# CliMA/ClimateParameterizations.jl

Measured on AMD Instinct MI355X. Metric: column-timesteps/sec (fwd+adjoint), 32-level wind-mixing NDE, higher is better.
Workload: dtype f32

## Files before the change

### climateparameterizations.jl_amd/csrc/engine_regtile.hip

```cpp
#include <cstdlib>
#include "engine_regtile.h"
#include "kernel_select.h"
#include "split_bf16.h"

typedef float f32x16 __attribute__((ext_vector_type(16)));

#ifdef COLNDE_STAMPS
__device__ unsigned long long g_rt_stamps[16];
#define RT_STAMP_DECL unsigned long long rs_t0 = 0, rs_acc[8] = {0, 0, 0, 0, 0, 0, 0, 0}; const unsigned long long rs_kk = __builtin_amdgcn_s_memtime(), rs_rr = __builtin_amdgcn_s_memrealtime()
#define RT_STAMP_BEGIN() do { __builtin_amdgcn_sched_barrier(0); rs_t0 = __builtin_amdgcn_s_memtime(); __builtin_amdgcn_sched_barrier(0); } while (0)
#define RT_STAMP(i) do { __builtin_amdgcn_sched_barrier(0); unsigned long long t_ = __builtin_amdgcn_s_memtime(); rs_acc[i] += t_ - rs_t0; rs_t0 = t_; __builtin_amdgcn_sched_barrier(0); } while (0)
#define RT_STAMP_FLUSH() do { if (blockIdx.x == 0 && threadIdx.x == 0) { for (int q_ = 0; q_ < 8; q_++) g_rt_stamps[q_] = rs_acc[q_]; g_rt_stamps[8] = __builtin_amdgcn_s_memtime() - rs_kk; g_rt_stamps[9] = __builtin_amdgcn_s_memrealtime() - rs_rr; } } while (0)
#else
#define RT_STAMP_DECL
#define RT_STAMP_BEGIN()
#define RT_STAMP(i)
#define RT_STAMP_FLUSH()
#endif
typedef float f32x4v __attribute__((ext_vector_type(4)));
typedef float f32x2v __attribute__((ext_vector_type(2)));

#define RHO0(r) (((r) & 3) + 8 * ((r) >> 2))
#ifndef RT16_WAVES
#define RT16_WAVES 8
#endif
#ifndef RT_ADJ_CH
#define RT_ADJ_CH 8
#endif
#ifndef RT_ZRICH
#define RT_ZRICH 0
#endif
#ifndef RT_Z2TAPE
#define RT_Z2TAPE 0
#endif
#define RT_TAPEZ_HALF (21 * 256)
#define RT_Z2OFF ((RT_ZRICH ? 2 : 1) * RT_TAPEZ_HALF)
#define RT_TAPEZ (RT_Z2OFF + (RT_Z2TAPE ? 9 * 256 : 0))
#define RT_TAPE2 (20 * 256)

__device__ __forceinline__ f32x16 mfma32(float a, float b, f32x16 c) {
    return __builtin_amdgcn_mfma_f32_32x32x2f32(a, b, c, 0, 0, 0);
}

__device__ __forceinline__ float xchg32(float from_hi, float from_lo, int h) {
    const auto r = __builtin_amdgcn_permlane32_swap(__float_as_uint(from_hi), __float_as_uint(from_lo), false, false);
    return __uint_as_float(h ? r[0] : r[1]);
}
__device__ __forceinline__ float swap32(float x, int h) { return xchg32(x, x, h); }

__device__ __forceinline__ f32x16 shift_down(const f32x16 T, int h, float below) {
    f32x16 o;
#pragma unroll
    for (int g = 0; g < 4; g++) {
        const float recv = xchg32(g > 0 ? T[(4 * g + 15) & 15] : 0.0f, T[4 * g + 3], h);
        o[4 * g] = (h == 0 && g == 0) ? below : recv;
        o[4 * g + 1] = T[4 * g];
        o[4 * g + 2] = T[4 * g + 1];
        o[4 * g + 3] = T[4 * g + 2];
    }
    return o;
}

__device__ __forceinline__ f32x16 shift_up(const f32x16 T, int h, float above) {
    f32x16 o;
#pragma unroll
    for (int g = 0; g < 4; g++) {
        const float recv = xchg32(T[4 * g], g < 3 ? T[(4 * g + 4) & 15] : 0.0f, h);
        o[4 * g + 3] = (h == 1 && g == 3) ? above : recv;
        o[4 * g] = T[4 * g + 1];
        o[4 * g + 1] = T[4 * g + 2];
        o[4 * g + 2] = T[4 * g + 3];
    }
    return o;
}

template <int ACT>
__device__ __forceinline__ float rt_act(float z) {
    if (ACT == COLNDE_ACT_RELU) return fmaxf(z, 0.0f);
    if (ACT == COLNDE_ACT_MISH) {
        const float e = __expf(__builtin_amdgcn_fmed3f(z, -3.0e38f, 20.0f));
        const float n = e * (e + 2.0f);
        return z * fast_div(n, n + 2.0f);
    }
    if (ACT == COLNDE_ACT_SWISH) return fast_div(z, 1.0f + __expf(-z));
    if (ACT == COLNDE_ACT_TANH) { const float e = __expf(2.0f * fminf(fmaxf(z, -15.0f), 15.0f)); return 1.0f - fast_div(2.0f, 1.0f + e); }
    if (ACT == COLNDE_ACT_LEAKYRELU) return z > 0.0f ? z : 0.01f * z;
    return z;
}

template <int ACT>
__device__ __forceinline__ f32x16 act_tile(f32x16 z) {
    f32x16 o;
#pragma unroll
    for (int r = 0; r < 16; r++) o[r] = rt_act<ACT>(z[r]);
    return o;
}

struct RtBases {
    int a1[5];
    int a2;
    int a3;
};

__device__ __forceinline__ RtBases rt_bases(int lane) {
    const int i = lane & 31, h = lane >> 5;
    const int r_i = (i & 3) + 4 * (i >> 3), h_i = (i >> 2) & 1;
    RtBases b;
#pragma unroll
    for (int mt = 0; mt < 5; mt++) {
        const int G = min(mt * 16 + r_i, 74);
        const int row = (G / 25) * 50 + 2 * (G % 25) + h_i;
        b.a1[mt] = RT_W1C + row * RT_LD1 + 4 * h;
    }
    b.a2 = RT_W2C + ((r_i < 10) ? 2 * r_i + h_i : 0) * RT_LD2 + h;
    b.a3 = RT_W3C + (i - 1) * RT_LD3 + h;
    return b;
}

#define RT_SCHED_FENCE() __builtin_amdgcn_sched_barrier(0x00F)
#define RT_SCHED_HARD() __builtin_amdgcn_sched_barrier(0)

template <int N, int CH, class AF, class BF, class FF>
__device__ __forceinline__ f32x16 rt_chain_fill(const float* wl, f32x16 acc, AF aidx, BF bval, FF fill) {
    float a[2][CH];
#pragma unroll
    for (int u = 0; u < CH; u++)
        if (u < N) a[0][u] = wl[aidx(u)];
    RT_SCHED_FENCE();
#pragma unroll
    for (int c = 0; c * CH < N; c++) {
#pragma unroll
        for (int u = 0; u < CH; u++)
            if ((c + 1) * CH + u < N) a[(c + 1) & 1][u] = wl[aidx((c + 1) * CH + u)];
        fill(c);
#pragma unroll
        for (int u = 0; u < CH; u++)
            if (c * CH + u < N) acc = mfma32(a[c & 1][u], bval(c * CH + u), acc);
        RT_SCHED_FENCE();
    }
    return acc;
}

template <int N, int CH, class AF, class BF>
__device__ __forceinline__ f32x16 rt_chain(const float* wl, f32x16 acc, AF aidx, BF bval) {
    return rt_chain_fill<N, CH>(wl, acc, aidx, bval, [](int) {});
}

template <int ACT>
__device__ __forceinline__ void rt_mlp_forward(const float* wl, const RtBases& b, const f32x16 (&X)[3], int h, f32x16 (&O)[3]) {
    f32x16 A1[5];
#pragma unroll
    for (int mt = 0; mt < 5; mt++) {
        f32x16 acc;
#pragma unroll
        for (int r = 0; r < 16; r++) {
            const int G = mt * 16 + r;
            acc[r] = wl[RT_B1C + (G < 75 ? (G / 25) * 50 + 2 * (G % 25) : 150 + 2 * (G - 75)) + h];
        }
        const int base = b.a1[mt];
        A1[mt] = rt_chain_fill<48, 8>(wl, acc, [=](int s) { return base + (s >> 4) * 32 + RHO0(s & 15); },
                                      [&](int s) { return X[s >> 4][s & 15]; },
                                      [&](int c) {
                                          if (mt > 0) {
#pragma unroll
                                              for (int r = 0; r < 16; r++)
                                                  if (r / 3 == c) A1[mt > 0 ? mt - 1 : 0][r] = rt_act<ACT>(A1[mt > 0 ? mt - 1 : 0][r]);
                                          }
                                      });
    }
    f32x16 Z2[3];
#pragma unroll
    for (int n = 0; n < 3; n++) {
        f32x16 acc;
#pragma unroll
        for (int r = 0; r < 16; r++) acc[r] = r < 10 ? wl[RT_B2C + n * 20 + 2 * r + h] : 0.0f;
        const int base2 = b.a2 + n * 20 * RT_LD2;
        Z2[n] = rt_chain_fill<25, 5>(wl, acc, [=](int s) { return base2 + 2 * s; },
                                     [&](int s) { return A1[(25 * n + s) >> 4][(25 * n + s) & 15]; },
                                     [&](int c) {
                                         if (n == 0) {
#pragma unroll
                                             for (int r = 0; r < 16; r++)
                                                 if (r / 4 == c) A1[4][r] = rt_act<ACT>(A1[4][r]);
                                         } else {
#pragma unroll
                                             for (int r = 0; r < 10; r++)
                                                 if (r / 2 == c) Z2[n > 0 ? n - 1 : 0][r] = rt_act<ACT>(Z2[n > 0 ? n - 1 : 0][r]);
                                         }
// ... 505 lines not shown
    }
}

#define RT_DMA_AUX 2
#ifdef RT_PLAIN_TAPE_STORES
#define RT_NT_STORE4(p, v) (*reinterpret_cast<f32x4v*>(p) = (f32x4v)(v))
#define RT_NT_STORE1(p, v) (*(float*)(p) = (float)(v))
#else
#define RT_NT_STORE4(p, v) __builtin_nontemporal_store((f32x4v)(v), reinterpret_cast<f32x4v*>(p))
#define RT_NT_STORE1(p, v) __builtin_nontemporal_store((float)(v), (float*)(p))
#endif
#define RT_TAPE_LOAD4(p) __builtin_nontemporal_load(reinterpret_cast<const f32x4v*>(p))
#define RT_TB (32 * 36)
#define RT_LAM(e, lane) ((((e) >> 2) * 64 + (lane)) * 4 + ((e) & 3))
__device__ __forceinline__ f32x16 rt_transpose(float* tb, const f32x16 T, int wbase, int rbase) {
#pragma unroll
    for (int a = 0; a < 4; a++)
        *reinterpret_cast<f32x4v*>(tb + wbase + 8 * a) = (f32x4v){T[4 * a], T[4 * a + 1], T[4 * a + 2], T[4 * a + 3]};
    f32x16 o;
#pragma unroll
    for (int s = 0; s < 16; s++) o[s] = tb[rbase + 72 * s];
    return o;
}

__device__ __forceinline__ f32x16 rt_outer(f32x16 acc, const f32x16 TA, const f32x16 TB) {
#pragma unroll
    for (int s = 0; s < 16; s++) acc = mfma32(TA[s], TB[s], acc);
    return acc;
}

struct Bf3x2 { Bf3 b[2]; };
__device__ __forceinline__ Bf3x2 rt_split_tile(const f32x16 T) {
    Bf3x2 o;
#pragma unroll
    for (int b = 0; b < 2; b++) {
        float v[8];
#pragma unroll
        for (int u = 0; u < 8; u++) v[u] = T[8 * b + u];
        o.b[b] = bf3_split8(v);
    }
    return o;
}
__device__ __forceinline__ f32x16 rt_outer_split(f32x16 acc, const Bf3x2& A, const Bf3x2& B) {
    acc = mfma_bf3(A.b[0], B.b[0], acc);
    acc = mfma_bf3(A.b[1], B.b[1], acc);
    return acc;
}

__device__ __forceinline__ float rt_sum16(const f32x16 v) {
    float s = 0.0f;
#pragma unroll
    for (int r = 0; r < 16; r++) s += v[r];
    return s;
}

#define RT_NET_LO(mt) (((mt) * 16) / 25)
#define RT_NET_HI(mt) ((((mt) * 16 + 15) < 75 ? ((mt) * 16 + 15) : 74) / 25)
__host__ __device__ constexpr int rt_combo(int n, int mt) { return n == 0 ? mt : (n == 1 ? 1 + mt : 2 + mt); }

template <int ACT, bool ZT, bool SPLIT = false>
__global__ void __launch_bounds__(256)
rt_adjoint_kernel(DevModel m, const float* __restrict__ wimg, const float* __restrict__ bcs,
                  const float* __restrict__ save_times, int n_save, int substeps, const float* __restrict__ sol,
                  const float* __restrict__ truth, const float* __restrict__ tape, float* __restrict__ tape2,
                  const float* __restrict__ tapez ,
                  LossWeights lw, float* __restrict__ slab, int n_col) {
    static_assert(!SPLIT || ZT, "the split W1^T operands replace the fp32 W1 in LDS: no layer-1 recomputation");
    float* wl = rt_smem;
    if constexpr (SPLIT) {
        static_assert(RT_ASIMG_HM_WORDS + 576 <= RT_W2C, "the split W1^T operands must fit the fp32 W1's place");
        const u32x4* src = reinterpret_cast<const u32x4*>(wimg + RT_ASIMG_OFF);
        for (int e = threadIdx.x; e < (RT_ASIMG_HM_WORDS + 576) / 4; e += blockDim.x) reinterpret_cast<u32x4*>(rt_smem)[e] = src[e];
        for (int e = RT_W2C + threadIdx.x; e < RT_IMG_FLOATS; e += blockDim.x) wl[e] = wimg[e];
    } else {
        for (int e = threadIdx.x; e < RT_IMG_FLOATS; e += blockDim.x) wl[e] = wimg[e];
    }
    __syncthreads();
    const int lane = threadIdx.x & 63, wave = threadIdx.x >> 6;
    const int j = lane & 31, h = lane >> 5;
    const int tile = blockIdx.x * RT_WAVES + wave;
    if (tile * RT_COLS >= n_col) return;
    float* lam = rt_smem + ((RT_IMG_FLOATS + 3) & ~3) + wave * (3072 + RT_TB);
    float* tb = lam + 3072;
    const int col = tile * RT_COLS + j;
    const bool valid = col < n_col;
    const int i_ = lane & 31, r_i = (i_ & 3) + 4 * (i_ >> 3), h_i = (i_ >> 2) & 1;
    int a1n[2];
#pragma unroll
    for (int t = 0; t < 2; t++) a1n[t] = RT_W1C + (2 * min(t * 16 + r_i, 24) + h_i) * RT_LD1 + 4 * h;
    const int a2b = RT_W2C + ((r_i < 10) ? 2 * r_i + h_i : 0) * RT_LD2 + h;
    const int f2c = (r_i < 10) ? 2 * r_i + h_i : 20;
    const int b3T = RT_W3C + (4 * h - 1) * RT_LD3 + f2c;
    int b2T[2];
#pragma unroll
    for (int t = 0; t < 2; t++) b2T[t] = RT_W2C + h * RT_LD2 + ((t * 16 + r_i < 25) ? 2 * (t * 16 + r_i) + h_i : 50);
    const int b1T = RT_W1C + h * RT_LD1 + i_;
    const int wbase = j * 36 + 4 * h, rbase = h * 36 + i_;

    f32x16 gW3[3], gW2[3][2];
#pragma unroll
    for (int q = 0; q < 3; q++) { gW3[q] = (f32x16)(0.0f); gW2[q][0] = (f32x16)(0.0f); gW2[q][1] = (f32x16)(0.0f); }
    float b2acc[3] = {0, 0, 0}, b3acc[3] = {0, 0, 0};
    float sums[6] = {0, 0, 0, 0, 0, 0};
    RT_STAMP_DECL;
    f32x16 xb[3], X[3];
#pragma unroll
    for (int q = 0; q < 3; q++) xb[q] = (f32x16)(0.0f);
    f32x16 xbs[3];
#pragma unroll
    for (int q = 0; q < 3; q++) xbs[q] = (f32x16)(0.0f);
#pragma unroll
    for (int e = 0; e < 48; e++) lam[RT_LAM(e, lane)] = 0.0f;

    const int n_steps = (n_save - 1) * substeps;
    const float* tp = tape + (size_t)tile * n_steps * 4 * 3072 + lane * 4;
    float* tp2 = tape2 + (size_t)tile * n_steps * 4 * RT_TAPE2 + lane * 4;
    const float* tpz = ZT ? tapez + (size_t)tile * n_steps * 4 * RT_TAPEZ + lane * 4 : nullptr;

    auto inject = [&](int n, bool add) {
#pragma unroll
        for (int q = 0; q < 3; q++) {
            f32x16 d;
#pragma unroll
            for (int g = 0; g < 4; g++) {
                const size_t o = ((size_t)min(col, n_col - 1) * n_save + n) * 96 + q * 32 + 8 * g + 4 * h;
                const f32x4v a = *reinterpret_cast<const f32x4v*>(sol + o);
                const f32x4v b = *reinterpret_cast<const f32x4v*>(truth + o);
#pragma unroll
                for (int e = 0; e < 4; e++) d[4 * g + e] = valid ? a[e] - b[e] : 0.0f;
            }
            const f32x16 dd = shift_down(d, h, 0.0f);
            f32x16 gg;
#pragma unroll
            for (int r = 0; r < 16; r++) {
                gg[r] = (r == 0 && h == 0) ? 0.0f : (d[r] - dd[r]) * 32.0f;
                sums[q] += d[r] * d[r];
                sums[3 + q] += gg[r] * gg[r];
            }
            if (add) {
                const f32x16 gu_ = shift_up(gg, h, 0.0f);
#pragma unroll
                for (int r = 0; r < 16; r++)
                    lam[RT_LAM(q * 16 + r, lane)] += 2.0f * lw.w[q] * d[r] + 2.0f * lw.w[3 + q] * 32.0f * (gg[r] - gu_[r]);
            }
        }
    };
    inject(0, false);

    auto load_z1 = [&](int step, int st, int n, f32x16 (&Z)[2], f32x16 (&Dz)[2]) {
        size_t rec = (size_t)step * 4 + st;
#ifdef RT_ABL_Z1_CACHED
        { int z_ = 0; asm volatile("" : "+v"(z_)); rec = (size_t)z_; }
#endif
        const float* srcz = tpz + rec * RT_TAPEZ + n * 7 * 256;
#pragma unroll
        for (int grp = 0; grp < 7; grp++) {
            const f32x4v v = RT_TAPE_LOAD4(srcz + grp * 256);
#pragma unroll
            for (int e = 0; e < 4; e++)
                if (4 * grp + e < 25) Z[grp >> 2][(grp & 3) * 4 + e] = v[e];
        }
        if (RT_ZRICH) {
#pragma unroll
            for (int grp = 0; grp < 7; grp++) {
                const f32x4v v = RT_TAPE_LOAD4(srcz + RT_TAPEZ_HALF + grp * 256);
#pragma unroll
                for (int e = 0; e < 4; e++)
                    if (4 * grp + e < 25) Dz[grp >> 2][(grp & 3) * 4 + e] = v[e];
            }
        }
    };

    auto load_z2 = [&](int step, int st, int n, f32x16& Z) {
        const float* srcz = tpz + ((size_t)step * 4 + st) * RT_TAPEZ + RT_Z2OFF + n * 3 * 256;
#pragma unroll
        for (int grp = 0; grp < 3; grp++) {
            const f32x4v v = RT_TAPE_LOAD4(srcz + grp * 256);
#pragma unroll
            for (int e = 0; e < 4; e++) Z[4 * grp + e] = (4 * grp + e < 10) ? v[e] : 0.0f;
        }
#pragma unroll
        for (int r = 12; r < 16; r++) Z[r] = 0.0f;
    };

    auto load_x = [&](int step, int st) {
        const float* src = tp + ((size_t)step * 4 + st) * 3072;
#pragma unroll
        for (int q = 0; q < 3; q++)
#pragma unroll
            for (int g = 0; g < 4; g++) {
                const f32x4v v = RT_TAPE_LOAD4(src + (q * 4 + g) * 256);
                X[q][4 * g] = v[0]; X[q][4 * g + 1] = v[1]; X[q][4 * g + 2] = v[2]; X[q][4 * g + 3] = v[3];
            }
    };

    for (int iv = n_save - 2; iv >= 0; iv--) {
        const float dt = (save_times[iv + 1] - save_times[iv]) / (float)substeps;
        inject(iv + 1, true);
        for (int s = substeps - 1; s >= 0; s--) {
            const int step = iv * substeps + s;
#pragma nounroll
            for (int st = 3; st >= 0; st--) {
                const float cwl = (st == 0 || st == 3) ? dt / 6.0f : dt / 3.0f;
                const float cwx = st == 3 ? 0.0f : (st == 2 ? dt : 0.5f * dt);
                RT_STAMP_BEGIN();
                f32x16 A1[2], D1[2];
                f32x16 A1n[2], D1n[2];
#pragma unroll
                for (int r = 9; r < 16; r++) { A1[1][r] = 0.0f; D1[1][r] = 0.0f; A1n[1][r] = 0.0f; D1n[1][r] = 0.0f; }
                load_x(step, st);
                f32x16 dOk[3];
                {
                    f32x16 kb[3];
#pragma unroll
                    for (int q = 0; q < 3; q++)
#pragma unroll
                        for (int r = 0; r < 16; r++) kb[q][r] = cwl * lam[RT_LAM(q * 16 + r, lane)] + cwx * xb[q][r];
                    rt_physics_vjp(m, X, kb, h, xb);
#pragma unroll
                    for (int q = 0; q < 3; q++) dOk[q] = kb[q];
                }
                RT_STAMP(0);
                float* dst = tp2 + ((size_t)step * 4 + st) * RT_TAPE2;
                float carry[2] = {0.0f, 0.0f};
#pragma unroll
                for (int n = 0; n < 3; n++) {
                    const f32x16 dOn = dOk[n];
                    if (ZT) {
                        if (n == 0) {
                            load_z1(step, st, 0, A1, D1);
#ifdef COLNDE_STAMPS
                            asm volatile("s_waitcnt vmcnt(0)" ::: "memory");
                            RT_STAMP(7);
#endif
                            if (!RT_ZRICH) {
#pragma unroll
                                for (int G = 0; G < 24; G += 4) rt_act_pair4_at<ACT>(A1, D1, G);
                                rt_act_pair_at<ACT>(A1, D1, 24);
                            }
                        }
                    } else {
#pragma unroll
                        for (int t = 0; t < 2; t++) {
                            f32x16 acc;
#pragma unroll
                            for (int r = 0; r < 16; r++) acc[r] = (t * 16 + r < 25) ? wl[RT_B1C + n * 50 + 2 * (t * 16 + r) + h] : 0.0f;
                            const int base = a1n[t] + n * 50 * RT_LD1;
                            acc = rt_chain<48, RT_ADJ_CH>(wl, acc, [=](int k) { return base + (k >> 4) * 32 + RHO0(k & 15); },
                                                          [&](int k) { return X[k >> 4][k & 15]; });
#pragma unroll
                            for (int r = 0; r < 16; r++) {
                                float av = 0.0f, dv = 0.0f;
                                if (t * 16 + r < 25) rt_act_pair<ACT>(acc[r], av, dv);
                                A1[t][r] = av;
                                D1[t][r] = dv;
                            }
                        }
                    }
                    RT_STAMP(1);
                    f32x16 Z2;
                    if (ZT && RT_Z2TAPE) load_z2(step, st, n, Z2);
                    else {
                        f32x16 acc;
#pragma unroll
                        for (int r = 0; r < 16; r++) acc[r] = r < 10 ? wl[RT_B2C + n * 20 + 2 * r + h] : 0.0f;
                        const int base2 = a2b + n * 20 * RT_LD2;
                        Z2 = rt_chain<25, 5>(wl, acc, [=](int k) { return base2 + 2 * k; },
                                             [&](int k) { return A1[k >> 4][k & 15]; });
                    }
                    RT_STAMP(2);
                    {
#ifndef RT_ABL_NO_OUTER
                        const f32x16 TA = rt_transpose(tb, dOn, wbase, rbase);
                        b3acc[n] += rt_sum16(TA);
#endif
                        f32x16 A2;
#pragma unroll
                        for (int r = 0; r < 16; r += 4) {
                            f32x2v a0 = {0.0f, 0.0f}, d0 = {0.0f, 0.0f}, a1 = {0.0f, 0.0f}, d1 = {0.0f, 0.0f};
                            if (r < 8) rt_act_pair4<ACT>((f32x2v){Z2[r], Z2[r + 1]}, (f32x2v){Z2[r + 2], Z2[r + 3]}, a0, d0, a1, d1);
                            else if (r == 8) rt_act_pair2<ACT>((f32x2v){Z2[8], Z2[9]}, a0, d0);
                            A2[r] = a0.x; A2[r + 1] = a0.y; A2[r + 2] = a1.x; A2[r + 3] = a1.y;
                            Z2[r] = d0.x; Z2[r + 1] = d0.y; Z2[r + 2] = d1.x; Z2[r + 3] = d1.y;
                        }
#ifndef RT_ABL_NO_OUTER
                        const f32x16 TB = rt_transpose(tb, A2, wbase, rbase);
#ifdef RT_OUTER_SPLIT
                        if constexpr (SPLIT) gW3[n] = rt_outer_split(gW3[n], rt_split_tile(TA), rt_split_tile(TB));
                        else
#endif
                        gW3[n] = rt_outer(gW3[n], TA, TB);
#else
                        gW3[n][0] += A2[0];
#endif
                    }
                    {
                        const int base = b3T + n * 31 * RT_LD3;
                        const f32x16 da = rt_chain<16, 8>(wl, (f32x16)(0.0f), [=](int k) { return base + RHO0(k) * RT_LD3; },
                                                          [&](int k) { return dOn[k]; });
#pragma unroll
                        for (int r = 0; r < 16; r++) Z2[r] = da[r] * Z2[r];
                    }
                    RT_STAMP(3);
                    if (ZT && n < 2) load_z1(step, st, n + 1, A1n, D1n);
#ifndef RT_LPIPE
#define RT_LPIPE 1
#endif
                    u32x4 Lr[9];
                    const u32x4* lg = nullptr;
                    if constexpr (SPLIT) {
                        int lz = lane;
                        asm volatile("" : "+v"(lz));
                        lg = reinterpret_cast<const u32x4*>(wimg + RT_ASIMG_OFF + RT_ASIMG_L) + n * 9 * 64 + lz;
#pragma unroll
                        for (int u = 0; u < (RT_LPIPE ? 3 : 9); u++) Lr[u] = lg[u * 64];
                    }
#ifdef RT_ABL_NO_OUTER
                    gW2[n][0][0] += Z2[0] * A1[0][0]; gW2[n][1][0] += Z2[1] * A1[1][0];
#else
                    {
                        const f32x16 TA = rt_transpose(tb, Z2, wbase, rbase);
                        b2acc[n] += rt_sum16(TA);
#ifdef RT_OUTER_SPLIT
// ... 278 lines not shown
        read_half(0, 0);
        asm volatile("s_waitcnt lgkmcnt(0)" ::: "memory");
        issue(4, 0);
        issue(5, 1);
    }
    for (int Qb = 0; Qb < NQ; Qb += 4) {
#pragma unroll
        for (int u = 0; u < 2; u++) {
            const int cur = u;
            asm volatile("s_waitcnt vmcnt(16)" ::: "memory");
            read_half(cur ^ 1, 2 * (u ^ 1));
            __builtin_amdgcn_sched_barrier(0);
            Bf3 X[3];
#pragma unroll
            for (int q = 0; q < 3; q++) X[q] = bf3_split8(raw[cur][q]);
            __builtin_amdgcn_sched_barrier(0);
            asm volatile("s_waitcnt lgkmcnt(0)" ::: "memory");
            issue(Qb + 2 * u + 6, 2 * (u ^ 1));
            issue(Qb + 2 * u + 7, 2 * (u ^ 1) + 1);
            __builtin_amdgcn_sched_barrier(0);
#pragma unroll
            for (int mt = 0; mt < 5; mt++) {
                const Bf3 Z = bf3_split8(raw[cur][3 + mt]);
#pragma unroll
                for (int q = 0; q < 3; q++) gW1[mt][q] = mfma_bf3(Z, X[q], gW1[mt][q]);
                const float* z = raw[cur][3 + mt];
                b1acc[mt] += ((z[0] + z[1]) + (z[2] + z[3])) + ((z[4] + z[5]) + (z[6] + z[7]));
            }
            __builtin_amdgcn_sched_barrier(0);
        }
    }
    asm volatile("s_waitcnt vmcnt(0)" ::: "memory");
    float* out = slab_rows + (size_t)gw * (m.n_params + 8);
#pragma unroll
    for (int mt = 0; mt < 5; mt++) {
#pragma unroll
        for (int r = 0; r < 16; r++) {
            const int G = mt * 16 + r;
            if (G < 75) {
                const int n = G / 25, f = 2 * (G % 25) + h;
#pragma unroll
                for (int q = 0; q < 3; q++) out[n * m.net_size + m.w_off[0] + (q * 32 + j) * 50 + f] = gW1[mt][q][r];
            }
        }
        const float s1 = b1acc[mt] + swap32(b1acc[mt], h);
        const int r_j = (j & 3) + 4 * (j >> 3), h_j = (j >> 2) & 1;
        const int G = mt * 16 + r_j;
        if (h == 0 && G < 75) out[(G / 25) * m.net_size + m.b_off[0] + 2 * (G % 25) + h_j] = s1;
    }
}

typedef float f32x4t __attribute__((ext_vector_type(4)));

__device__ __forceinline__ f32x4t mfma16t(float a, float b, f32x4t c) {
    return __builtin_amdgcn_mfma_f32_16x16x4f32(a, b, c, 0, 0, 0);
}

__device__ __forceinline__ f32x4t mfma16_bf(u32x4 a, u32x4 b, f32x4t c) {
    return __builtin_amdgcn_mfma_f32_16x16x32_bf16(__builtin_bit_cast(bf16x8, a), __builtin_bit_cast(bf16x8, b), c, 0, 0, 0);
}
__device__ __forceinline__ f32x4t mfma16_bf3(const Bf3& a, const Bf3& b, f32x4t c) {
    c = mfma16_bf(a.m, b.m, c);
    c = mfma16_bf(a.l, b.h, c);
    c = mfma16_bf(a.h, b.l, c);
    c = mfma16_bf(a.m, b.h, c);
    c = mfma16_bf(a.h, b.m, c);
    c = mfma16_bf(a.h, b.h, c);
    return c;
}
__device__ __forceinline__ Bf3 rt16_ldA(const u32x4* simg, int G, int lane) {
    Bf3 a;
    a.h = simg[(G * 3 + 0) * 64 + lane];
    a.m = simg[(G * 3 + 1) * 64 + lane];
    a.l = simg[(G * 3 + 2) * 64 + lane];
    return a;
}

__device__ __forceinline__ float rot_dn16(float x, int lane) { return __shfl(x, (lane + 48) & 63); }
__device__ __forceinline__ float rot_up16(float x, int lane) { return __shfl(x, (lane + 16) & 63); }

struct V16 { f32x4t t[2]; };

__device__ __forceinline__ V16 shift_down16(const V16& T, int lane, float below) {
    const int g = lane >> 4;
    const float r0 = rot_dn16(T.t[0][3], lane), r1 = rot_dn16(T.t[1][3], lane);
    V16 o;
    o.t[0][0] = g == 0 ? below : r0;
    o.t[1][0] = g == 0 ? r0 : r1;
#pragma unroll
    for (int tau = 0; tau < 2; tau++) { o.t[tau][1] = T.t[tau][0]; o.t[tau][2] = T.t[tau][1]; o.t[tau][3] = T.t[tau][2]; }
    return o;
}

__device__ __forceinline__ V16 shift_up16(const V16& T, int lane, float above) {
    const int g = lane >> 4;
    const float r0 = rot_up16(T.t[0][0], lane), r1 = rot_up16(T.t[1][0], lane);
    V16 o;
    o.t[0][3] = g == 3 ? r1 : r0;
    o.t[1][3] = g == 3 ? above : r1;
#pragma unroll
    for (int tau = 0; tau < 2; tau++) { o.t[tau][0] = T.t[tau][1]; o.t[tau][1] = T.t[tau][2]; o.t[tau][2] = T.t[tau][3]; }
    return o;
}

template <int N, int CH, class AF, class BF>
__device__ __forceinline__ f32x4t rt16_chain(const float* wl, f32x4t acc, AF aidx, BF bval) {
    float a[2][CH];
#pragma unroll
    for (int u = 0; u < CH; u++)
        if (u < N) a[0][u] = wl[aidx(u)];
    RT_SCHED_FENCE();
    __builtin_amdgcn_s_setprio(1);
#pragma unroll
    for (int c = 0; c * CH < N; c++) {
#pragma unroll
        for (int u = 0; u < CH; u++)
            if ((c + 1) * CH + u < N) a[(c + 1) & 1][u] = wl[aidx((c + 1) * CH + u)];
#pragma unroll
        for (int u = 0; u < CH; u++)
            if (c * CH + u < N) acc = mfma16t(a[c & 1][u], bval(c * CH + u), acc);
        RT_SCHED_FENCE();
    }
    __builtin_amdgcn_s_setprio(0);
    return acc;
}

template <int N, int CH, int NV, class AF, class BF, class FF>
__device__ __forceinline__ f32x4t rt16_chain_fill(const float* wl, f32x4t acc, AF aidx, BF bval, FF fill) {
    float a[2][CH];
#pragma unroll
    for (int u = 0; u < CH; u++)
        if (u < N) a[0][u] = wl[aidx(u)];
    RT_SCHED_HARD();
    fill();
#pragma unroll
    for (int c = 0; c * CH < N; c++) {
#pragma unroll
        for (int u = 0; u < CH; u++)
            if ((c + 1) * CH + u < N) a[(c + 1) & 1][u] = wl[aidx((c + 1) * CH + u)];
#pragma unroll
        for (int u = 0; u < CH; u++)
            if (c * CH + u < N) acc = mfma16t(a[c & 1][u], bval(c * CH + u), acc);
    }
#pragma unroll
    for (int i = 0; i < N; i++) {
        __builtin_amdgcn_sched_group_barrier(0x008, 1, 0);
        __builtin_amdgcn_sched_group_barrier(0x100, 1, 0);
        __builtin_amdgcn_sched_group_barrier(0x402, NV, 0);
    }
    RT_SCHED_HARD();
    return acc;
}

#ifndef RT_Z1_DWORD
#define RT_Z1_DWORD 1
#endif
__device__ __forceinline__ void rt16_tape_z1(float* oz , float (&zpre)[40], const f32x4t z, int tt, int g) {
#pragma unroll
    for (int r = 0; r < 4; r++) {
        const int Q = 4 * tt + r, qq = Q % 13, net = Q / 13;
        if (Q >= 39) continue;
        if (RT_Z1_DWORD) {
            if (qq < 12 || g < 2) oz[(net * 7 + (qq >> 1)) * 256 + ((2 * qq) & 3)] = z[r];
            continue;
        }
        zpre[Q] = z[r];
        if (qq == 12) {
            if (g < 2) oz[(net * 7 + 6) * 256] = z[r];
        } else if ((qq & 3) == 3) {
            const int Q0 = Q - 3;
            const auto s02 = __builtin_amdgcn_permlane32_swap(__float_as_uint(zpre[Q0]), __float_as_uint(zpre[Q0 + 2]), false, false);
            const auto s13 = __builtin_amdgcn_permlane32_swap(__float_as_uint(zpre[Q0 + 1]), __float_as_uint(zpre[Q0 + 3]), false, false);
            const f32x4v v = {__uint_as_float(s02[0]), __uint_as_float(s02[1]), __uint_as_float(s13[0]), __uint_as_float(s13[1])};
            *reinterpret_cast<f32x4v*>(oz - (g >> 1) + (net * 7 + ((qq - 3) >> 1) + (g >> 1)) * 256) = v;
        }
    }
}

template <int ACT, bool SPLIT = false>
__global__ void __launch_bounds__(512)
rt16_forward_kernel(DevModel m, const float* __restrict__ wimg, const float* __restrict__ x0, const float* __restrict__ bcs,
                    const float* __restrict__ save_times, int n_save, int substeps, float* __restrict__ sol,
                    float* __restrict__ tape, float* __restrict__ tapez, int n_col) {
    float* wl = rt_smem;
    const float* bl = wl;
    const u32x4* simg = reinterpret_cast<const u32x4*>(rt_smem);
    if constexpr (SPLIT) {
        const unsigned* src = reinterpret_cast<const unsigned*>(wimg + RT_SIMG_OFF);
        unsigned* dst = reinterpret_cast<unsigned*>(rt_smem);
        for (int e = threadIdx.x; e < RT_SIMG_WORDS / 4; e += blockDim.x)
            reinterpret_cast<u32x4*>(dst)[e] = reinterpret_cast<const u32x4*>(src)[e];
        for (int e = threadIdx.x; e < RT_IMG_FLOATS - RT_B1C; e += blockDim.x) wl[RT_SIMG_WORDS + e] = wimg[RT_B1C + e];
        bl = wl + RT_SIMG_WORDS - RT_B1C;
    } else {
        for (int e = threadIdx.x; e < RT_IMG_FLOATS; e += blockDim.x) wl[e] = wimg[e];
    }
    __syncthreads();
    const int lane = threadIdx.x & 63, wave = threadIdx.x >> 6;
    const int j = lane & 15, g = lane >> 4;
    const int wt = blockIdx.x * (blockDim.x >> 6) + wave;
    const int tile32 = wt >> 1, half = wt & 1;
    if (tile32 * 32 >= n_col) return;
    const int col = wt * 16 + j;
    const bool valid = col < n_col;
    const int colc = min(col, n_col - 1);
    const int i_ = lane & 15, g_i = i_ >> 2, r_i = i_ & 3;
    int a1b[10];
#pragma unroll
    for (int t = 0; t < 10; t++) {
        const int Q = 4 * t + r_i, f = 4 * (Q % 13) + g_i;
        const int row = (Q < 39 && f < 50) ? (Q / 13) * 50 + f : 0;
        a1b[t] = RT_W1C + row * RT_LD1 + 4 * g;
    }
    int a2b[2], a2l[2], a3b[2];
#pragma unroll
    for (int u = 0; u < 2; u++) {
        const int Q2 = 4 * u + r_i;
        const int row2 = Q2 < 5 ? 4 * Q2 + g_i : 0;
        a2b[u] = RT_W2C + row2 * RT_LD2 + g;
        a2l[u] = RT_W2C + row2 * RT_LD2 + (g < 2 ? 48 + g : 50);
        a3b[u] = RT_W3C + (16 * u + i_ - 1) * RT_LD3 + g;
    }
    RtBC bc;
    float bc5;
    {
        const float* bp = bcs + (size_t)colc * 6;
        bc.b[0] = bp[0]; bc.t[0] = bp[1]; bc.b[1] = bp[2]; bc.t[1] = bp[3]; bc.b[2] = bp[4]; bc5 = bp[5];
        bc.t[2] = bc5;
    }
    V16 Xn[3];
#pragma unroll
    for (int q = 0; q < 3; q++)
#pragma unroll
        for (int tau = 0; tau < 2; tau++) {
            const f32x4v v = *reinterpret_cast<const f32x4v*>(x0 + (size_t)colc * 96 + q * 32 + 16 * tau + 4 * g);
            Xn[q].t[tau] = v;
            if (sol && valid) *reinterpret_cast<f32x4v*>(sol + ((size_t)col * n_save) * 96 + q * 32 + 16 * tau + 4 * g) = v;
        }
    const int n_steps = (n_save - 1) * substeps;
    RT_STAMP_DECL;
#ifdef COLNDE_STAMPS_FWD
    const unsigned long long rs_k0 = __builtin_amdgcn_s_memtime(), rs_r0 = __builtin_amdgcn_s_memrealtime();
#endif
    float* tp = tape ? tape + (size_t)tile32 * n_steps * 4 * 3072 + ((g >> 1) * 64 + j + 16 * half + 32 * (g & 1)) * 4 : nullptr;
    float* tz = tapez ? tapez + (size_t)tile32 * n_steps * 4 * RT_TAPEZ + (j + 16 * half + 32 * (g & 1)) * 4 + (g >> 1) : nullptr;
    const float Nz = 32.0f;
    struct { float cU, sU, cV, sV, cB, sB, kE, oE, cE, nA, nB, f0, f1, f2; } pc;
    {
        const float L2E = 1.4426950408889634f;
        pc.cU = m.sig_u * Nz; pc.sU = m.sig_u * m.eps; pc.cV = m.sig_v * Nz; pc.sV = m.sig_v * m.eps; pc.cB = m.B * Nz; pc.sB = m.B * m.eps;
        pc.kE = 2.0f * m.inv_dRi * L2E; pc.oE = -2.0f * m.Ric * m.inv_dRi * L2E; pc.cE = 30.0f * L2E;
        pc.nA = -0.5f * m.nu_minus; pc.nB = m.nu0 + 0.5f * m.nu_minus;
        pc.f0 = -m.cs[0] * Nz; pc.f1 = -m.cs[1] * Nz; pc.f2 = -m.cs[2] * m.inv_Pr * Nz;
    }
    int step = 0;
    for (int iv = 0; iv < n_save - 1; iv++) {
        const float t0 = save_times[iv];
        const float dt = (save_times[iv + 1] - t0) / (float)substeps;
        for (int s = 0; s < substeps; s++, step++) {
            const float ts = t0 + (float)s * dt;
            V16 Xs[3], Kacc[3];
#pragma unroll
            for (int q = 0; q < 3; q++) { Xs[q] = Xn[q]; Kacc[q].t[0] = (f32x4t)(0.0f); Kacc[q].t[1] = (f32x4t)(0.0f); }
#pragma nounroll
            for (int st = 0; st < 4; st++) {
                const float ca = st == 0 ? 0.0f : (st == 3 ? 1.0f : 0.5f);
                const float cb = (st == 0 || st == 3) ? 1.0f / 6.0f : 1.0f / 3.0f;
                RT_STAMP_BEGIN();
                if (tp) {
                    float* o = tp + ((size_t)step * 4 + st) * 3072;
#pragma unroll
                    for (int q = 0; q < 3; q++)
#pragma unroll
                        for (int tau = 0; tau < 2; tau++) *reinterpret_cast<f32x4v*>(o + (q * 4 + 2 * tau) * 256) = Xs[q].t[tau];
                }
                bc.t[2] = rt_top_flux(m, bc5, ts + ca * dt);
                RT_STAMP(0);
                f32x4t A1[10];
                float zpre[40];
                int lz = lane;
                if constexpr (SPLIT) asm volatile("" : "+v"(lz));
                if constexpr (SPLIT) {
#pragma unroll
                    for (int t = 0; t < 10; t++)
#pragma unroll
                        for (int r = 0; r < 4; r++) {
                            const int Q = 4 * t + r;
                            A1[t][r] = Q < 39 ? bl[RT_B1C + (Q / 13) * 50 + min(4 * (Q % 13) + g, 49)] : 0.0f;
                        }
                    Bf3 Apf = rt16_ldA(simg, 0, lz);
#pragma unroll
                    for (int q = 0; q < 3; q++) {
                        const float x8[8] = {Xs[q].t[0][0], Xs[q].t[0][1], Xs[q].t[0][2], Xs[q].t[0][3], Xs[q].t[1][0], Xs[q].t[1][1], Xs[q].t[1][2], Xs[q].t[1][3]};
                        const Bf3 XB = bf3_split8(x8);
#pragma unroll
                        for (int t = 0; t < 10; t++) {
                            const Bf3 Ac = Apf;
                            const int nx = q * 10 + t + 1;
                            if (nx < 30) Apf = rt16_ldA(simg, 3 * (nx % 10) + nx / 10, lz);
                            auto finish = [&](int tt) {
                                if (tz && !RT_ZRICH) rt16_tape_z1(tz + ((size_t)step * 4 + st) * RT_TAPEZ, zpre, A1[tt], tt, g);
#pragma unroll
                                for (int r = 0; r < 4; r++) asm volatile("" : "+v"(A1[tt][r]));
                                if (RT_ZRICH && tz) {
                                    f32x2v a0, d0, a1, d1;
                                    rt_act_pair4<ACT>((f32x2v){A1[tt][0], A1[tt][1]}, (f32x2v){A1[tt][2], A1[tt][3]}, a0, d0, a1, d1);
                                    A1[tt] = (f32x4t){a0.x, a0.y, a1.x, a1.y};
                                    const float dd[4] = {d0.x, d0.y, d1.x, d1.y};
                                    float* oz = tz + ((size_t)step * 4 + st) * RT_TAPEZ;
#pragma unroll
                                    for (int r = 0; r < 4; r++) {
                                        const int Q = 4 * tt + r, qq = Q % 13;
                                        if (Q < 39 && (qq < 12 || g < 2)) {
                                            oz[((Q / 13) * 7 + (qq >> 1)) * 256 + ((2 * qq) & 3)] = A1[tt][r];
                                            oz[RT_TAPEZ_HALF + ((Q / 13) * 7 + (qq >> 1)) * 256 + ((2 * qq) & 3)] = dd[r];
                                        }
                                    }
                                } else
                                A1[tt] = rt_act4<ACT>(A1[tt]);
#pragma unroll
                                for (int r = 0; r < 4; r++) asm volatile("" : "+v"(A1[tt][r]));
                            };
                            if (q == 2) RT_SCHED_HARD();
                            __builtin_amdgcn_s_setprio(1);
                            A1[t] = mfma16_bf3(Ac, XB, A1[t]);
                            __builtin_amdgcn_s_setprio(0);
                            if (q == 2) {
                                if (t > 0) {
                                    finish(t - 1);
#pragma unroll
                                    for (int u = 0; u < 6; u++) {
                                        __builtin_amdgcn_sched_group_barrier(0x008, 1, 0);
                                        __builtin_amdgcn_sched_group_barrier(0x402, 9, 0);
                                    }
                                }
                                RT_SCHED_HARD();
                                if (t == 9) finish(9);
                            } else
                                RT_SCHED_FENCE();
                        }
                    }
                } else {
                auto finish1 = [&](int tt) {
                    if (tz && !RT_ZRICH) rt16_tape_z1(tz + ((size_t)step * 4 + st) * RT_TAPEZ, zpre, A1[tt], tt, g);
#pragma unroll
                    for (int r = 0; r < 4; r++) asm volatile("" : "+v"(A1[tt][r]));
                    if (RT_ZRICH && tz) {
                        f32x2v a0, d0, a1, d1;
                        rt_act_pair4<ACT>((f32x2v){A1[tt][0], A1[tt][1]}, (f32x2v){A1[tt][2], A1[tt][3]}, a0, d0, a1, d1);
                        A1[tt] = (f32x4t){a0.x, a0.y, a1.x, a1.y};
                        const float dd[4] = {d0.x, d0.y, d1.x, d1.y};
                        float* oz = tz + ((size_t)step * 4 + st) * RT_TAPEZ;
#pragma unroll
                        for (int r = 0; r < 4; r++) {
                            const int Q = 4 * tt + r, qq = Q % 13;
                            if (Q < 39 && (qq < 12 || g < 2)) {
                                oz[((Q / 13) * 7 + (qq >> 1)) * 256 + ((2 * qq) & 3)] = A1[tt][r];
                                oz[RT_TAPEZ_HALF + ((Q / 13) * 7 + (qq >> 1)) * 256 + ((2 * qq) & 3)] = dd[r];
                            }
                        }
                    } else
                    A1[tt] = rt_act4<ACT>(A1[tt]);
#pragma unroll
                    for (int r = 0; r < 4; r++) asm volatile("" : "+v"(A1[tt][r]));
                };
#pragma unroll
                for (int t = 0; t < 10; t++) {
                    f32x4t acc;
#pragma unroll
                    for (int r = 0; r < 4; r++) {
                        const int Q = 4 * t + r;
                        acc[r] = Q < 39 ? wl[RT_B1C + (Q / 13) * 50 + min(4 * (Q % 13) + g, 49)] : 0.0f;
                    }
                    const int base = a1b[t];
#ifndef RT16_FWD_FILL
                    acc = rt16_chain<24, 8>(wl, acc, [=](int k) { return base + (k >> 3) * 32 + ((k >> 2) & 1) * 16 + (k & 3); },
                                            [&](int k) { return Xs[k >> 3].t[(k >> 2) & 1][k & 3]; });
                    A1[t] = acc;
                    finish1(t);
#else
                    acc = rt16_chain_fill<24, 8, 2>(wl, acc, [=](int k) { return base + (k >> 3) * 32 + ((k >> 2) & 1) * 16 + (k & 3); },
                                                    [&](int k) { return Xs[k >> 3].t[(k >> 2) & 1][k & 3]; }, [&] { if (t > 0) finish1(t - 1); });
                    A1[t] = acc;
                    if (t == 9) finish1(9);
#endif
                }
                }
                RT_STAMP(1);
                V16 O[3];
#pragma unroll
                for (int n = 0; n < 3; n++) {
                    f32x4t A2[2];
                    Bf3 HB[2];
                    if constexpr (SPLIT) {
#pragma unroll
                        for (int c = 0; c < 2; c++) {
                            float a8[8];
#pragma unroll
                            for (int e = 0; e < 8; e++) a8[e] = 8 * c + e < 13 ? A1[(13 * n + 8 * c + e) >> 2][(13 * n + 8 * c + e) & 3] : 0.0f;
                            HB[c] = bf3_split8(a8);
                        }
                    }
#pragma unroll
                    for (int u = 0; u < 2; u++) {
                        f32x4t acc;
#pragma unroll
                        for (int r = 0; r < 4; r++) acc[r] = (4 * u + r < 5) ? bl[RT_B2C + n * 20 + 4 * (4 * u + r) + g] : 0.0f;
                        if constexpr (SPLIT) {
                            const Bf3 Aa = rt16_ldA(simg, 30 + 4 * n + 2 * u, lz), Ab = rt16_ldA(simg, 30 + 4 * n + 2 * u + 1, lz);
                            __builtin_amdgcn_s_setprio(1);
                            acc = mfma16_bf3(Aa, HB[0], acc);
                            acc = mfma16_bf3(Ab, HB[1], acc);
                            __builtin_amdgcn_s_setprio(0);
                            RT_SCHED_FENCE();
                        } else {
                        const int base = a2b[u] + n * 20 * RT_LD2, basel = a2l[u] + n * 20 * RT_LD2;
                        acc = rt16_chain<13, 13>(wl, acc, [=](int k) { return k < 12 ? base + 4 * k : basel; },
                                                 [&](int k) { return A1[(13 * n + k) >> 2][(13 * n + k) & 3]; });
                        }
                        if (RT_Z2TAPE && tz) {
                            float* oz = tz + ((size_t)step * 4 + st) * RT_TAPEZ + RT_Z2OFF;
#pragma unroll
                            for (int r = 0; r < 4; r++) {
                                const int Q2 = 4 * u + r;
                                if (Q2 < 5) oz[(3 * n + (Q2 >> 1)) * 256 + ((2 * Q2) & 3)] = acc[r];
                            }
                        }
                        A2[u] = rt_act4<ACT>(acc);
                    }
                    Bf3 GB;
                    if constexpr (SPLIT) {
                        const float a8[8] = {A2[0][0], A2[0][1], A2[0][2], A2[0][3], A2[1][0], 0.0f, 0.0f, 0.0f};
                        GB = bf3_split8(a8);
                    }
#pragma unroll
                    for (int v = 0; v < 2; v++) {
                        f32x4t acc;
#pragma unroll
                        for (int r = 0; r < 4; r++) acc[r] = bl[RT_B3C + n * 32 + 16 * v + 4 * g + r];
                        if constexpr (SPLIT) {
                            const Bf3 Aa = rt16_ldA(simg, 42 + 2 * n + v, lz);
                            __builtin_amdgcn_s_setprio(1);
                            O[n].t[v] = mfma16_bf3(Aa, GB, acc);
                            __builtin_amdgcn_s_setprio(0);
                            RT_SCHED_FENCE();
                        } else {
                        const int base = a3b[v] + n * 31 * RT_LD3;
                        O[n].t[v] = rt16_chain<5, 5>(wl, acc, [=](int k) { return base + 4 * k; },
                                                     [&](int k) { return A2[k >> 2][k & 3]; });
                        }
                    }
                }
                RT_STAMP(2);
                V16 F[3];
                {
                    V16 Ud, Vd, Td;
                    if (m.mpp || m.ca) {
                        Ud = shift_down16(Xs[0], lane, 0.0f); Vd = shift_down16(Xs[1], lane, 0.0f); Td = shift_down16(Xs[2], lane, 0.0f);
                    }
                    if (m.mpp) {
#pragma unroll
                        for (int tau = 0; tau < 2; tau++)
#pragma unroll
                            for (int r = 0; r < 4; r += 2) {
                                const f32x2v dU = {Xs[0].t[tau][r] - Ud.t[tau][r], Xs[0].t[tau][r + 1] - Ud.t[tau][r + 1]};
                                const f32x2v dV = {Xs[1].t[tau][r] - Vd.t[tau][r], Xs[1].t[tau][r + 1] - Vd.t[tau][r + 1]};
                                const f32x2v dT = {Xs[2].t[tau][r] - Td.t[tau][r], Xs[2].t[tau][r + 1] - Td.t[tau][r + 1]};
                                const f32x2v a1 = dU * pc.cU + pc.sU, a2 = dV * pc.cV + pc.sV;
                                const f32x2v s2 = a2 * a2 + a1 * a1;
                                f32x2v rS;
                                rS.x = __builtin_amdgcn_rcpf(s2.x);
                                rS.y = __builtin_amdgcn_rcpf(s2.y);
                                const f32x2v arg = ((dT * pc.cB + pc.sB) * rS) * pc.kE + pc.oE;
                                f32x2v e;
                                e.x = __builtin_amdgcn_exp2f(__builtin_amdgcn_fmed3f(arg.x, -pc.cE, pc.cE));
                                e.y = __builtin_amdgcn_exp2f(__builtin_amdgcn_fmed3f(arg.y, -pc.cE, pc.cE));
                                const f32x2v e1 = e + 1.0f;
                                f32x2v rc;
                                rc.x = __builtin_amdgcn_rcpf(e1.x);
                                rc.y = __builtin_amdgcn_rcpf(e1.y);
                                const f32x2v nu = (rc * -2.0f + 1.0f) * pc.nA + pc.nB;
                                const f32x2v o0 = {O[0].t[tau][r], O[0].t[tau][r + 1]}, o1 = {O[1].t[tau][r], O[1].t[tau][r + 1]},
                                             o2 = {O[2].t[tau][r], O[2].t[tau][r + 1]};
                                const f32x2v f0 = (nu * dU) * pc.f0 + o0, f1 = (nu * dV) * pc.f1 + o1, f2 = (nu * dT) * pc.f2 + o2;
                                F[0].t[tau][r] = f0.x; F[0].t[tau][r + 1] = f0.y;
                                F[1].t[tau][r] = f1.x; F[1].t[tau][r + 1] = f1.y;
                                F[2].t[tau][r] = f2.x; F[2].t[tau][r + 1] = f2.y;
                            }
                        if (g == 0) {
#pragma unroll
                            for (int k = 0; k < 3; k++) F[k].t[0][0] = m.zero_w ? bc.b[k] - m.s0[k] : bc.b[k];
                        }
                    } else
#pragma unroll
                    for (int tau = 0; tau < 2; tau++)
#pragma unroll
                        for (int r = 0; r < 4; r++) {
                            const bool in = !(tau == 0 && r == 0 && g == 0);
                            float f0 = in ? O[0].t[tau][r] : 0.0f, f1 = in ? O[1].t[tau][r] : 0.0f, f2 = in ? O[2].t[tau][r] : 0.0f;
                            if (!m.zero_w && !in) { f0 = bc.b[0]; f1 = bc.b[1]; f2 = bc.b[2]; }
                            if (m.ca && in) {
                                const float gT = (Xs[2].t[tau][r] - Td.t[tau][r]) * Nz;
                                f2 -= m.cs[2] * m.kappa * fminf(0.0f, gT);
                            }
                            F[0].t[tau][r] = f0; F[1].t[tau][r] = f1; F[2].t[tau][r] = f2;
                        }
                }
#pragma unroll
                for (int k = 0; k < 3; k++) {
                    const float top = m.zero_w ? bc.t[k] - m.s0[k] : bc.t[k];
                    const V16 Fu = shift_up16(F[k], lane, top);
#pragma unroll
                    for (int tau = 0; tau < 2; tau++)
#pragma unroll
                        for (int r = 0; r < 4; r++) {
                            float v = -m.A[k] * (Fu.t[tau][r] - F[k].t[tau][r]);
                            if (k == 0) v += m.cor_u * (m.sig_v * Xs[1].t[tau][r] + m.mu_v);
                            if (k == 1) v -= m.cor_v * (m.sig_u * Xs[0].t[tau][r] + m.mu_u);
                            F[k].t[tau][r] = v;
                        }
                }
                RT_STAMP(3);
                const float can = st == 2 ? 1.0f : 0.5f;
#pragma unroll
                for (int q = 0; q < 3; q++)
#pragma unroll
                    for (int tau = 0; tau < 2; tau++) {
                        Kacc[q].t[tau] += cb * F[q].t[tau];
                        Xs[q].t[tau] = Xn[q].t[tau] + (can * dt) * F[q].t[tau];
                    }
                RT_STAMP(4);
            }
#pragma unroll
            for (int q = 0; q < 3; q++)
#pragma unroll
                for (int tau = 0; tau < 2; tau++) Xn[q].t[tau] += dt * Kacc[q].t[tau];
            if (s == substeps - 1 && sol && valid) {
#pragma unroll
                for (int q = 0; q < 3; q++)
#pragma unroll
                    for (int tau = 0; tau < 2; tau++)
                        *reinterpret_cast<f32x4v*>(sol + ((size_t)col * n_save + iv + 1) * 96 + q * 32 + 16 * tau + 4 * g) = Xn[q].t[tau];
            }
        }
    }
#ifdef COLNDE_STAMPS_FWD
    rs_acc[6] = __builtin_amdgcn_s_memtime() - rs_k0;
    rs_acc[7] = __builtin_amdgcn_s_memrealtime() - rs_r0;
    RT_STAMP_FLUSH();
#endif
}

template <int ACT>
__device__ __forceinline__ void rt16_act_pair(const f32x4t z, f32x4t& a, f32x4t& d) {
    const f32x2v z0 = {z[0], z[1]}, z1 = {z[2], z[3]};
    f32x2v a0, d0, a1, d1;
    rt_act_pair4<ACT>(z0, z1, a0, d0, a1, d1);
    a = (f32x4t){a0.x, a0.y, a1.x, a1.y};
    d = (f32x4t){d0.x, d0.y, d1.x, d1.y};
}

#define RT16S_RREC ((3 * 12 + 18) * 256)
template <int ACT, bool RICH>
__global__ void __launch_bounds__(192)
rt16s_forward_kernel(DevModel m, const float* __restrict__ wimg, const float* __restrict__ x0, const float* __restrict__ bcs,
                     const float* __restrict__ save_times, int n_save, int substeps, float* __restrict__ sol,
                     float* __restrict__ t16_tape, float* __restrict__ t16_ztape, int n_col) {
    float* wl = rt_smem;
    for (int e = threadIdx.x; e < RT_IMG_FLOATS; e += 192) wl[e] = wimg[e];
    f32x4v* ex = reinterpret_cast<f32x4v*>(rt_smem + ((RT_IMG_FLOATS + 3) & ~3));
    __syncthreads();
    const int lane = threadIdx.x & 63;
    const int n = __builtin_amdgcn_readfirstlane(threadIdx.x >> 6);
    const int j = lane & 15, g = lane >> 4;
// ... 1732 lines not shown
```

Baseline: 188.6 million.

## Store layer-1 tape as whole f32x4 records matching forward register layout

Changes the z1 tape layout so the forward kernel writes each A1 register quad as one 16-byte vector store instead of scattered dword stores or permlane-swapped packing. The adjoint load_z1 is rewritten to gather from the new layout, reading the tiles that overlap each net and picking out valid elements. The per-record size shrinks slightly and the Z2 tape offset is adjusted for the new base pointer. This cuts forward store instruction count but may load more unused data on the adjoint side.

Result: faster. 190.9 million, median of 6 (+1.2%).

```diff
diff --git a/climateparameterizations.jl_amd/csrc/engine_regtile.hip b/climateparameterizations.jl_amd/csrc/engine_regtile.hip
--- a/climateparameterizations.jl_amd/csrc/engine_regtile.hip
+++ b/climateparameterizations.jl_amd/csrc/engine_regtile.hip
@@ -33,7 +33,7 @@
 #ifndef RT_Z2TAPE
 #define RT_Z2TAPE 0
 #endif
-#define RT_TAPEZ_HALF (21 * 256)
+#define RT_TAPEZ_HALF (20 * 256)
 #define RT_Z2OFF ((RT_ZRICH ? 2 : 1) * RT_TAPEZ_HALF)
 #define RT_TAPEZ (RT_Z2OFF + (RT_Z2TAPE ? 9 * 256 : 0))
 #define RT_TAPE2 (20 * 256)
@@ -845,23 +845,22 @@
 #ifdef RT_ABL_Z1_CACHED
         { int z_ = 0; asm volatile("" : "+v"(z_)); rec = (size_t)z_; }
 #endif
-        const float* srcz = tpz + rec * RT_TAPEZ + n * 7 * 256;
-#pragma unroll
-        for (int grp = 0; grp < 7; grp++) {
-            const f32x4v v = RT_TAPE_LOAD4(srcz + grp * 256);
-#pragma unroll
-            for (int e = 0; e < 4; e++)
-                if (4 * grp + e < 25) Z[grp >> 2][(grp & 3) * 4 + e] = v[e];
-        }
-        if (RT_ZRICH) {
-#pragma unroll
-            for (int grp = 0; grp < 7; grp++) {
-                const f32x4v v = RT_TAPE_LOAD4(srcz + RT_TAPEZ_HALF + grp * 256);
-#pragma unroll
-                for (int e = 0; e < 4; e++)
-                    if (4 * grp + e < 25) Dz[grp >> 2][(grp & 3) * 4 + e] = v[e];
-            }
-        }
+        const float* srcz = tpz + rec * RT_TAPEZ;
+        auto fill = [&](const float* src, f32x16 (&T)[2]) {
+#pragma unroll
+            for (int t = (13 * n) >> 2; t <= (13 * n + 12) >> 2; t++)
+#pragma unroll
+                for (int c = 0; c < 2; c++) {
+                    const f32x4v v = RT_TAPE_LOAD4(src + (2 * t + c) * 256);
+#pragma unroll
+                    for (int e = 0; e < 4; e++) {
+                        const int G = 2 * (4 * t + e - 13 * n) + c;
+                        if ((4 * t + e) / 13 == n && G < 25) T[G >> 4][G & 15] = v[e];
+                    }
+                }
+        };
+        fill(srcz, Z);
+        if (RT_ZRICH) fill(srcz + RT_TAPEZ_HALF, Dz);
     };
 
     auto load_z2 = [&](int step, int st, int n, f32x16& Z) {
@@ -1446,31 +1445,6 @@
     return acc;
 }
 
-#ifndef RT_Z1_DWORD
-#define RT_Z1_DWORD 1
-#endif
-__device__ __forceinline__ void rt16_tape_z1(float* oz , float (&zpre)[40], const f32x4t z, int tt, int g) {
-#pragma unroll
-    for (int r = 0; r < 4; r++) {
-        const int Q = 4 * tt + r, qq = Q % 13, net = Q / 13;
-        if (Q >= 39) continue;
-        if (RT_Z1_DWORD) {
-            if (qq < 12 || g < 2) oz[(net * 7 + (qq >> 1)) * 256 + ((2 * qq) & 3)] = z[r];
-            continue;
-        }
-        zpre[Q] = z[r];
-        if (qq == 12) {
-            if (g < 2) oz[(net * 7 + 6) * 256] = z[r];
-        } else if ((qq & 3) == 3) {
-            const int Q0 = Q - 3;
-            const auto s02 = __builtin_amdgcn_permlane32_swap(__float_as_uint(zpre[Q0]), __float_as_uint(zpre[Q0 + 2]), false, false);
-            const auto s13 = __builtin_amdgcn_permlane32_swap(__float_as_uint(zpre[Q0 + 1]), __float_as_uint(zpre[Q0 + 3]), false, false);
-            const f32x4v v = {__uint_as_float(s02[0]), __uint_as_float(s02[1]), __uint_as_float(s13[0]), __uint_as_float(s13[1])};
-            *reinterpret_cast<f32x4v*>(oz - (g >> 1) + (net * 7 + ((qq - 3) >> 1) + (g >> 1)) * 256) = v;
-        }
-    }
-}
-
 template <int ACT, bool SPLIT = false>
 __global__ void __launch_bounds__(512)
 rt16_forward_kernel(DevModel m, const float* __restrict__ wimg, const float* __restrict__ x0, const float* __restrict__ bcs,
@@ -1537,7 +1511,7 @@
     const unsigned long long rs_k0 = __builtin_amdgcn_s_memtime(), rs_r0 = __builtin_amdgcn_s_memrealtime();
 #endif
     float* tp = tape ? tape + (size_t)tile32 * n_steps * 4 * 3072 + ((g >> 1) * 64 + j + 16 * half + 32 * (g & 1)) * 4 : nullptr;
-    float* tz = tapez ? tapez + (size_t)tile32 * n_steps * 4 * RT_TAPEZ + (j + 16 * half + 32 * (g & 1)) * 4 + (g >> 1) : nullptr;
+    float* tz = tapez ? tapez + (size_t)tile32 * n_steps * 4 * RT_TAPEZ + ((g >> 1) * 64 + j + 16 * half + 32 * (g & 1)) * 4 : nullptr;
     const float Nz = 32.0f;
     struct { float cU, sU, cV, sV, cB, sB, kE, oE, cE, nA, nB, f0, f1, f2; } pc;
     {
@@ -1571,7 +1545,6 @@
                 bc.t[2] = rt_top_flux(m, bc5, ts + ca * dt);
                 RT_STAMP(0);
                 f32x4t A1[10];
-                float zpre[40];
                 int lz = lane;
                 if constexpr (SPLIT) asm volatile("" : "+v"(lz));
                 if constexpr (SPLIT) {
@@ -1593,23 +1566,16 @@
                             const int nx = q * 10 + t + 1;
                             if (nx < 30) Apf = rt16_ldA(simg, 3 * (nx % 10) + nx / 10, lz);
                             auto finish = [&](int tt) {
-                                if (tz && !RT_ZRICH) rt16_tape_z1(tz + ((size_t)step * 4 + st) * RT_TAPEZ, zpre, A1[tt], tt, g);
+                                float* oz = tz ? tz + ((size_t)step * 4 + st) * RT_TAPEZ + 2 * tt * 256 : nullptr;
+                                if (tz && !RT_ZRICH) *reinterpret_cast<f32x4v*>(oz) = A1[tt];
 #pragma unroll
                                 for (int r = 0; r < 4; r++) asm volatile("" : "+v"(A1[tt][r]));
                                 if (RT_ZRICH && tz) {
                                     f32x2v a0, d0, a1, d1;
                                     rt_act_pair4<ACT>((f32x2v){A1[tt][0], A1[tt][1]}, (f32x2v){A1[tt][2], A1[tt][3]}, a0, d0, a1, d1);
                                     A1[tt] = (f32x4t){a0.x, a0.y, a1.x, a1.y};
-                                    const float dd[4] = {d0.x, d0.y, d1.x, d1.y};
-                                    float* oz = tz + ((size_t)step * 4 + st) * RT_TAPEZ;
-#pragma unroll
-                                    for (int r = 0; r < 4; r++) {
-                                        const int Q = 4 * tt + r, qq = Q % 13;
-                                        if (Q < 39 && (qq < 12 || g < 2)) {
-                                            oz[((Q / 13) * 7 + (qq >> 1)) * 256 + ((2 * qq) & 3)] = A1[tt][r];
-                                            oz[RT_TAPEZ_HALF + ((Q / 13) * 7 + (qq >> 1)) * 256 + ((2 * qq) & 3)] = dd[r];
-                                        }
-                                    }
+                                    *reinterpret_cast<f32x4v*>(oz) = A1[tt];
+                                    *reinterpret_cast<f32x4v*>(oz + RT_TAPEZ_HALF) = (f32x4v){d0.x, d0.y, d1.x, d1.y};
                                 } else
                                 A1[tt] = rt_act4<ACT>(A1[tt]);
 #pragma unroll
@@ -1636,23 +1602,16 @@
                     }
                 } else {
                 auto finish1 = [&](int tt) {
-                    if (tz && !RT_ZRICH) rt16_tape_z1(tz + ((size_t)step * 4 + st) * RT_TAPEZ, zpre, A1[tt], tt, g);
+                    float* oz = tz ? tz + ((size_t)step * 4 + st) * RT_TAPEZ + 2 * tt * 256 : nullptr;
+                    if (tz && !RT_ZRICH) *reinterpret_cast<f32x4v*>(oz) = A1[tt];
 #pragma unroll
                     for (int r = 0; r < 4; r++) asm volatile("" : "+v"(A1[tt][r]));
                     if (RT_ZRICH && tz) {
                         f32x2v a0, d0, a1, d1;
                         rt_act_pair4<ACT>((f32x2v){A1[tt][0], A1[tt][1]}, (f32x2v){A1[tt][2], A1[tt][3]}, a0, d0, a1, d1);
                         A1[tt] = (f32x4t){a0.x, a0.y, a1.x, a1.y};
-                        const float dd[4] = {d0.x, d0.y, d1.x, d1.y};
-                        float* oz = tz + ((size_t)step * 4 + st) * RT_TAPEZ;
-#pragma unroll
-                        for (int r = 0; r < 4; r++) {
-                            const int Q = 4 * tt + r, qq = Q % 13;
-                            if (Q < 39 && (qq < 12 || g < 2)) {
-                                oz[((Q / 13) * 7 + (qq >> 1)) * 256 + ((2 * qq) & 3)] = A1[tt][r];
-                                oz[RT_TAPEZ_HALF + ((Q / 13) * 7 + (qq >> 1)) * 256 + ((2 * qq) & 3)] = dd[r];
-                            }
-                        }
+                        *reinterpret_cast<f32x4v*>(oz) = A1[tt];
+                        *reinterpret_cast<f32x4v*>(oz + RT_TAPEZ_HALF) = (f32x4v){d0.x, d0.y, d1.x, d1.y};
                     } else
                     A1[tt] = rt_act4<ACT>(A1[tt]);
 #pragma unroll
@@ -1713,7 +1672,7 @@
                                                  [&](int k) { return A1[(13 * n + k) >> 2][(13 * n + k) & 3]; });
                         }
                         if (RT_Z2TAPE && tz) {
-                            float* oz = tz + ((size_t)step * 4 + st) * RT_TAPEZ + RT_Z2OFF;
+                            float* oz = tz + ((size_t)step * 4 + st) * RT_TAPEZ + RT_Z2OFF - (g >> 1) * 255;
 #pragma unroll
                             for (int r = 0; r < 4; r++) {
                                 const int Q2 = 4 * u + r;
```
